# NightShade99/Self-Supervised-Vision

Measured on NVIDIA B200. Metric: ntxent_fwd_bwd_samples_per_s, higher is better.
Workload: dtype f16

## Files before the change

self-supervised-vision_b200/csrc/ntxent.cu:

```cuda
#include "sim_host.cuh"

using namespace ssvb;

namespace {

struct NtxPlan {
  int64_t n_glob, m, mpad, d, dpad;
  int mode;
  int normalize;
  float c, shift;
  float prescale;
  float wscale;
  float pos_c;
};

int make_plan(NtxPlan& pl, int64_t n_glob, int64_t d, int normalize, float temperature) {
  if (n_glob <= 0 || d <= 0 || !(temperature > 0.f)) return SSVB_ERR_INVALID;
  if (d % 4) return SSVB_ERR_ALIGNMENT;
  if (d > 256) return SSVB_ERR_UNSUPPORTED;
  if (2 * n_glob > (1 << 30)) return SSVB_ERR_UNSUPPORTED;
  pl.n_glob = n_glob;
  pl.m = 2 * n_glob;
  pl.mpad = sim_mpad(pl.m);
  pl.d = d;
  pl.dpad = sim_dpad(d);
  pl.normalize = normalize ? 1 : 0;
  const float c = SSVB_LOG2E / temperature;
  pl.mode = (normalize && 2.f * c <= 64.f) ? SIM_NTX_FIXED : SIM_NTX_ONLINE;
  if (pl.mode == SIM_NTX_FIXED) {
    pl.prescale = sqrtf(c);
    pl.c = 1.f;
    pl.shift = 0.f;
    pl.pos_c = 1.f;
    int k = 0;
    while ((int64_t{2} << k) <= pl.m) ++k;
    k -= 4;
    if (k < 0) k = 0;
    if (k > 14) k = 14;
    pl.wscale = static_cast<float>(1 << k);
  } else {
    pl.prescale = 1.f;
    pl.c = c;
    pl.shift = c;
    pl.pos_c = c;
    pl.wscale = 1.f;
  }
  return SSVB_OK;
}

struct SavedLayout {
  __nv_bfloat16* zhat;
  float* inv_norm;
  float* stat;
  size_t bytes;
};
SavedLayout saved_layout(void* base, int64_t mpad, int64_t dpad) {
  Carver c(base);
  SavedLayout s;
  s.zhat = c.take<__nv_bfloat16>(mpad * dpad);
  s.inv_norm = c.take<float>(mpad);
  s.stat = c.take<float>(mpad);
  s.bytes = c.used();
  return s;
}

struct WsLayout {
  float* pos;
  float* part_m;
  float* part_l;
  float* block_sums;
  unsigned int* counter;
  float* dacc;
  size_t bytes;
};
WsLayout ws_layout(void* base, int64_t local_rows, int64_t row_blocks, int64_t cols, int64_t dpad) {
  Carver c(base);
  WsLayout w;
  const int64_t lr = round_up(local_rows, 256);
  SimParams p{};
  p.row_blocks = static_cast<int>(row_blocks);
  p.cols = static_cast<int>(cols);
  plan_chunks(p, sim_fwd_bn(dpad), sim_fwd_min_tiles(dpad));
  size_t part_elems = static_cast<size_t>(4 * p.nchunks + 2) * lr;
  if (part_elems < static_cast<size_t>(sim_mpad(cols))) part_elems = sim_mpad(cols);
  w.pos = c.take<float>(lr);
  w.part_m = c.take<float>(part_elems);
  w.part_l = c.take<float>(part_elems);
  w.block_sums = c.take<float>(ceil_div(lr, 256) + 8);
  w.counter = c.take<unsigned int>(4);
  w.dacc = c.take<float>(lr * dpad);
  w.bytes = c.used();
  return w;
}

__global__ void ntx_grad_finish_kernel(const float* __restrict__ zi, const float* __restrict__ zj, int64_t ldi,
                                       int64_t ldj, int n_view, int d, int row0,
                                       const float* __restrict__ dacc, int ld_dacc,
                                       const __nv_bfloat16* __restrict__ zhat, int dpad,
                                       const float* __restrict__ inv_norm, int normalize, float inv_m_tau,
                                       const float* __restrict__ grad_out, float* __restrict__ dzi,
                                       float* __restrict__ dzj, int64_t ld_dzi, int64_t ld_dzj,
                                       float acc_scale, float zp_scale) {
  const int lrow = (blockIdx.x * blockDim.x + threadIdx.x) >> 5, lane = threadIdx.x & 31;
  if (lrow >= 2 * n_view) return;
  const int view = lrow >= n_view;
  const int r = lrow - view * n_view;
  const int a_glob = row0 + lrow;
  const int partner = view ? a_glob - n_view : a_glob + n_view;
  const float* z = view ? zj + static_cast<int64_t>(r) * ldj : zi + static_cast<int64_t>(r) * ldi;
  float* out = view ? dzj + static_cast<int64_t>(r) * ld_dzj : dzi + static_cast<int64_t>(r) * ld_dzi;
  const float scale = inv_m_tau * __ldg(grad_out);
  const float inv = normalize ? inv_norm[lrow] : 1.f;
  float g[2][4] = {{0.f, 0.f, 0.f, 0.f}, {0.f, 0.f, 0.f, 0.f}}, zh[2][4] = {{0.f, 0.f, 0.f, 0.f}, {0.f, 0.f, 0.f, 0.f}};
  float dot = 0.f;
#pragma unroll
  for (int it = 0; it < 2; ++it) {
    const int k = it * 128 + lane * 4;
    if (k < d) {
      const float4 acc = *reinterpret_cast<const float4*>(dacc + static_cast<int64_t>(lrow) * ld_dacc + k);
      const uint2 pz = *reinterpret_cast<const uint2*>(zhat + static_cast<int64_t>(partner) * dpad + k);
      const float2 p01 = unpack_h2(pz.x, normalize != 0), p23 = unpack_h2(pz.y, normalize != 0);
      const float4 zz = *reinterpret_cast<const float4*>(z + k);
      const float za = -2.f * zp_scale;
      g[it][0] = fmaf(acc.x, acc_scale, za * p01.x) * scale;
      g[it][1] = fmaf(acc.y, acc_scale, za * p01.y) * scale;
      g[it][2] = fmaf(acc.z, acc_scale, za * p23.x) * scale;
      g[it][3] = fmaf(acc.w, acc_scale, za * p23.y) * scale;
      zh[it][0] = zz.x * inv; zh[it][1] = zz.y * inv; zh[it][2] = zz.z * inv; zh[it][3] = zz.w * inv;
    }
    dot += g[it][0] * zh[it][0] + g[it][1] * zh[it][1] + g[it][2] * zh[it][2] + g[it][3] * zh[it][3];
  }
  if (normalize) {
    dot = warp_sum(dot);
#pragma unroll
    for (int it = 0; it < 2; ++it)
#pragma unroll
      for (int i = 0; i < 4; ++i) g[it][i] = (g[it][i] - dot * zh[it][i]) * inv;
  }
#pragma unroll
  for (int it = 0; it < 2; ++it) {
    const int k = it * 128 + lane * 4;
    if (k < d) *reinterpret_cast<float4*>(out + k) = make_float4(g[it][0], g[it][1], g[it][2], g[it][3]);
  }
}

int check_rows(const void* p, int64_t ld) {
  if (!p) return SSVB_ERR_INVALID;
  if ((reinterpret_cast<uintptr_t>(p) & 15) || (ld & 3)) return SSVB_ERR_ALIGNMENT;
  return SSVB_OK;
}

void fill_sim_params_rows(SimParams& p, const NtxPlan& pl, int nseg, int64_t seg_rows, int64_t s0, int64_t s1) {
  p = SimParams{};
  p.opf16 = pl.normalize ? 1 : 0;
  p.nseg = nseg;
  p.seg_rows = static_cast<int>(seg_rows);
  p.seg_start[0] = static_cast<int>(s0);
  p.seg_start[1] = static_cast<int>(s1);
  p.bps = static_cast<int>(ceil_div(seg_rows, 128));
  p.row_blocks = nseg * p.bps;
  p.cols = static_cast<int>(pl.m);
  p.c = pl.c;
  p.shift = pl.shift;
}

}

extern "C" {

int64_t ssvb_ntxent_dpad(int64_t d) { return sim_dpad(d); }
int64_t ssvb_ntxent_mpad(int64_t n_global) { return sim_mpad(2 * n_global); }

size_t ssvb_ntxent_saved_bytes(int64_t n, int64_t d) {
  if (n <= 0 || d <= 0) return 0;
  return saved_layout(nullptr, sim_mpad(2 * n), sim_dpad(d)).bytes;
}
size_t ssvb_ntxent_workspace_bytes(int64_t n, int64_t d) {
  if (n <= 0 || d <= 0) return 0;
  return ws_layout(nullptr, 2 * n, ceil_div(2 * n, 128), 2 * n, sim_dpad(d)).bytes;
}

int ssvb_ntxent_fwd(const float* zi, const float* zj, int64_t n, int64_t d, int64_t ld_zi, int64_t ld_zj,
                    int normalize, float temperature, float* loss, void* saved, void* workspace,
                    size_t workspace_bytes, void* stream) {
  SSVB_TRY(check_device_sm100());
  NtxPlan pl;
  SSVB_TRY(make_plan(pl, n, d, normalize, temperature));
  SSVB_TRY(check_rows(zi, ld_zi));
  SSVB_TRY(check_rows(zj, ld_zj));
  if (!loss || !saved || !workspace) return SSVB_ERR_INVALID;
  if (workspace_bytes < ssvb_ntxent_workspace_bytes(n, d)) return SSVB_ERR_WORKSPACE;
  cudaStream_t s = static_cast<cudaStream_t>(stream);
  SavedLayout sv = saved_layout(saved, pl.mpad, pl.dpad);
  WsLayout ws = ws_layout(workspace, pl.m, ceil_div(pl.m, 128), pl.m, pl.dpad);

  if (pl.mpad > pl.m)
    SSVB_CUDA(cudaMemsetAsync(sv.zhat + pl.m * pl.dpad, 0, (pl.mpad - pl.m) * pl.dpad * sizeof(__nv_bfloat16), s));
  {
    const int wpb = 8;
    pair_prep_kernel<<<static_cast<unsigned>(ceil_div(n, wpb)), wpb * 32, 0, s>>>(
        zi, zj, static_cast<int>(n), static_cast<int>(d), ld_zi, ld_zj, normalize, normalize ? 1 : 0, sv.zhat,
        sv.zhat + n * pl.dpad,
        static_cast<int>(pl.dpad), sv.inv_norm, sv.inv_norm + n, ws.pos, ws.pos + n, -1, pl.prescale, ws.counter);
    SSVB_LAUNCH_CHECK();
  }
  SimParams p;
  fill_sim_params_rows(p, pl, 1, pl.m, 0, 0);
  plan_chunks(p, sim_fwd_bn(pl.dpad), sim_fwd_min_tiles(pl.dpad));
  p.part_m = ws.part_m;
  p.part_l = ws.part_l;
  p.part_stride = static_cast<int>(round_up(pl.m, 256));
#ifdef SSVB_DBG_TIMING
  if (const char* e = getenv("SSVB_DBG_PTR")) p.dbg = reinterpret_cast<unsigned long long*>(strtoull(e, nullptr, 0));
#endif
  SSVB_TRY(launch_sim_fwd(pl.mode, sv.zhat, pl.mpad, sv.zhat, pl.mpad, pl.dpad, p, s));
  {
    const unsigned grid = static_cast<unsigned>(ceil_div(pl.m, 256));
    const float scale = 1.f / static_cast<float>(pl.m);
    if (pl.mode == SIM_NTX_FIXED)
      lse_finalize_kernel<SIM_NTX_FIXED><<<grid, 256, 0, s>>>(ws.part_m, ws.part_l, 4 * p.nchunks, p.part_stride,
                                                            static_cast<int>(pl.m), ws.pos, pl.c, pl.shift,
                                                            sv.stat, nullptr, ws.block_sums, ws.counter, scale, loss,
                                                            nullptr, nullptr, 0, 0, pl.wscale);
    else
      lse_finalize_kernel<SIM_NTX_ONLINE><<<grid, 256, 0, s>>>(ws.part_m, ws.part_l, 4 * p.nchunks, p.part_stride,
                                                             static_cast<int>(pl.m), ws.pos, pl.c, pl.shift,
                                                             sv.stat, nullptr, ws.block_sums, ws.counter, scale, loss);
    SSVB_LAUNCH_CHECK();
    if (pl.mpad > pl.m) {
      const float padv = pl.mode == SIM_NTX_FIXED ? 0.f : 1e30f;
      fill_kernel<<<static_cast<unsigned>(ceil_div(pl.mpad - pl.m, 256)), 256, 0, s>>>(sv.stat + pl.m,
                                                                                       pl.mpad - pl.m, padv);
      SSVB_LAUNCH_CHECK();
    }
  }
  return SSVB_OK;
}

int ssvb_ntxent_bwd(const float* zi, const float* zj, int64_t n, int64_t d, int64_t ld_zi, int64_t ld_zj,
                    int normalize, float temperature, const float* grad_out, const void* saved, float* dzi,
                    float* dzj, int64_t ld_dzi, int64_t ld_dzj, void* workspace, size_t workspace_bytes,
                    void* stream) {
  SSVB_TRY(check_device_sm100());
  NtxPlan pl;
  SSVB_TRY(make_plan(pl, n, d, normalize, temperature));
  SSVB_TRY(check_rows(zi, ld_zi));
  SSVB_TRY(check_rows(zj, ld_zj));
  SSVB_TRY(check_rows(dzi, ld_dzi));
  SSVB_TRY(check_rows(dzj, ld_dzj));
  if (!grad_out || !saved || !workspace) return SSVB_ERR_INVALID;
  if (workspace_bytes < ssvb_ntxent_workspace_bytes(n, d)) return SSVB_ERR_WORKSPACE;
  cudaStream_t s = static_cast<cudaStream_t>(stream);
  SavedLayout sv = saved_layout(const_cast<void*>(saved), pl.mpad, pl.dpad);
  WsLayout ws = ws_layout(workspace, pl.m, ceil_div(pl.m, 128), pl.m, pl.dpad);

  SimParams p;
  fill_sim_params_rows(p, pl, 1, pl.m, 0, 0);
  plan_chunks(p, 128, 8);
  p.rowstat = sv.stat;
  p.colstat = sv.stat;
  p.dacc = ws.dacc;
  p.ld_dacc = static_cast<int>(pl.dpad);
  p.use_atomic = p.nchunks > 1;
#ifdef SSVB_DBG_TIMING
  if (const char* e = getenv("SSVB_DBG_PTR")) p.dbg = reinterpret_cast<unsigned long long*>(strtoull(e, nullptr, 0));
#endif
  if (p.use_atomic) SSVB_CUDA(cudaMemsetAsync(ws.dacc, 0, pl.m * pl.dpad * sizeof(float), s));
  SSVB_TRY(launch_sim_bwd(pl.mode, sv.zhat, pl.mpad, sv.zhat, pl.mpad, pl.dpad, p, s));
  {
    const int wpb = 8;
    ntx_grad_finish_kernel<<<static_cast<unsigned>(ceil_div(pl.m, wpb)), wpb * 32, 0, s>>>(
        zi, zj, ld_zi, ld_zj, static_cast<int>(n), static_cast<int>(d), 0, ws.dacc,
        static_cast<int>(pl.dpad), sv.zhat, static_cast<int>(pl.dpad), sv.inv_norm, normalize,
        1.f / (static_cast<float>(pl.m) * temperature), grad_out, dzi, dzj, ld_dzi, ld_dzj,
        1.f / (pl.wscale * pl.prescale), 1.f / pl.prescale);
    SSVB_LAUNCH_CHECK();
  }
  return SSVB_OK;
}

size_t ssvb_ntxent_dist_workspace_bytes(int64_t world, int64_t n_local, int64_t d) {
  if (world <= 0 || n_local <= 0 || d <= 0) return 0;
  return ws_layout(nullptr, 2 * n_local, ceil_div(2 * n_local, 128), 2 * n_local * world, sim_dpad(d)).bytes;
}

namespace {
int dist_check(int64_t world, int64_t rank, int64_t n_local) {
  if (world <= 0 || rank < 0 || rank >= world || n_local <= 0) return SSVB_ERR_INVALID;
  return SSVB_OK;
}
}

int ssvb_ntxent_dist_prep(const float* zi, const float* zj, int64_t n_local, int64_t d, int64_t ld_zi,
                          int64_t ld_zj, int normalize, float temperature, int64_t world, int64_t rank,
                          void* zhat_all, float* inv_norm_local, float* pos_local, void* stream) {
  SSVB_TRY(check_device_sm100());
  SSVB_TRY(dist_check(world, rank, n_local));
  NtxPlan pl;
  SSVB_TRY(make_plan(pl, n_local * world, d, normalize, temperature));
  SSVB_TRY(check_rows(zi, ld_zi));
  SSVB_TRY(check_rows(zj, ld_zj));
  if (!zhat_all || !inv_norm_local || !pos_local) return SSVB_ERR_INVALID;
  cudaStream_t s = static_cast<cudaStream_t>(stream);
  __nv_bfloat16* zh = static_cast<__nv_bfloat16*>(zhat_all);
  if (pl.mpad > pl.m)
    SSVB_CUDA(cudaMemsetAsync(zh + pl.m * pl.dpad, 0, (pl.mpad - pl.m) * pl.dpad * sizeof(__nv_bfloat16), s));
  const int64_t row0 = rank * 2 * n_local;
  const int wpb = 8;
// ... 440 lines not shown
```

self-supervised-vision_b200/csrc/sim_host.cuh:

```cuda
#pragma once
#include "host_util.h"
#include "sim_kernels.cuh"

namespace ssvb {

inline int64_t sim_dpad(int64_t d) { return d <= 128 ? round_up(d, 64) : 256; }
inline int64_t sim_mpad(int64_t m) { return round_up(m, 256); }
inline int sim_fwd_bn(int64_t dpad) { return dpad > 128 ? 128 : kFwdBN; }
inline int sim_fwd_min_tiles(int64_t dpad) { return 1024 / sim_fwd_bn(dpad); }

inline void plan_chunks(SimParams& p, int BN, int min_tiles) {
  p.col_tiles = static_cast<int>(ceil_div(p.cols, BN));
  const int sms = num_sms();
  const int max_ch = p.col_tiles / min_tiles > 1 ? p.col_tiles / min_tiles : 1;
  int best = 1;
  double best_score = -1.0;
  for (int nch = 1; nch <= max_ch && nch <= 256; ++nch) {
    const int tpc = static_cast<int>(ceil_div(p.col_tiles, nch));
    const int real = static_cast<int>(ceil_div(p.col_tiles, tpc));
    if (real != nch) continue;
    const int64_t units = static_cast<int64_t>(p.row_blocks) * nch;
    const int64_t waves = ceil_div(units, sms);
    const double eff = static_cast<double>(p.row_blocks) * p.col_tiles / (static_cast<double>(waves) * sms * tpc);
    const double score = eff - 0.002 * nch;
    if (score > best_score) {
      best_score = score;
      best = nch;
    }
  }
  p.tiles_per_chunk = static_cast<int>(ceil_div(p.col_tiles, best));
  p.nchunks = static_cast<int>(ceil_div(p.col_tiles, p.tiles_per_chunk));
}

template <int KB, int MODE, bool OPF16 = false>
int launch_sim_fwd_t(const CUtensorMap& tmA, const CUtensorMap& tmB, const SimParams& p, cudaStream_t s) {
  auto kern = sim_fwd_kernel<KB, MODE, OPF16>;
  constexpr int smem = FwdCfg<KB>::SMEM;
  SSVB_TRY((set_smem_once<sim_fwd_kernel<KB, MODE, OPF16>>(smem)));
  const int nunits = p.row_blocks * p.nchunks;
  const int grid = nunits < num_sms() ? nunits : num_sms();
  const int slot = prof_begin(PROF_SIM_FWD, s);
  kern<<<grid, 640, smem, s>>>(tmA, tmB, p);
  prof_end(slot, s);
  SSVB_LAUNCH_CHECK();
  return SSVB_OK;
}
template <int KB, int MODE, bool OPF16 = false>
int launch_sim_bwd_t(const CUtensorMap& tmA, const CUtensorMap& tmB, const SimParams& p, cudaStream_t s) {
  auto kern = sim_bwd_kernel<KB, MODE, OPF16>;
  constexpr int smem = BwdCfg<KB>::SMEM;
  SSVB_TRY((set_smem_once<sim_bwd_kernel<KB, MODE, OPF16>>(smem)));
  const int nunits = p.row_blocks * p.nchunks;
  const int grid = nunits < num_sms() ? nunits : num_sms();
  const int slot = prof_begin(PROF_SIM_BWD, s);
  kern<<<grid, 640, smem, s>>>(tmA, tmB, p);
  prof_end(slot, s);
  SSVB_LAUNCH_CHECK();
  return SSVB_OK;
}

inline int launch_sim_fwd(int mode, const void* A, int64_t a_rows, const void* B, int64_t b_rows, int64_t dpad,
                          const SimParams& p, cudaStream_t s) {
  CUtensorMap tmA, tmB;
  SSVB_TRY(make_tmap_bf16(&tmA, A, a_rows, dpad, dpad, 128, p.opf16 != 0));
  SSVB_TRY(make_tmap_bf16(&tmB, B, b_rows, dpad, dpad, sim_fwd_bn(dpad), p.opf16 != 0));
  const int KB = static_cast<int>(dpad / 64);
#define SSVB_DISPATCH(KBV)                                                      \
  switch (mode) {                                                               \
    case SIM_NTX_FIXED:                                                         \
      if (p.opf16) return launch_sim_fwd_t<KBV, SIM_NTX_FIXED, true>(tmA, tmB, p, s);                   \
      return launch_sim_fwd_t<KBV, SIM_NTX_FIXED, false>(tmA, tmB, p, s);                               \
    case SIM_NTX_ONLINE:                                                        \
      if (p.opf16) return launch_sim_fwd_t<KBV, SIM_NTX_ONLINE, true>(tmA, tmB, p, s);                  \
      return launch_sim_fwd_t<KBV, SIM_NTX_ONLINE, false>(tmA, tmB, p, s);                              \
    case SIM_MOCO: return launch_sim_fwd_t<KBV, SIM_MOCO>(tmA, tmB, p, s);      \
    default: return SSVB_ERR_INVALID;                                           \
  }
  if (KB == 1) { SSVB_DISPATCH(1) }
  if (KB == 2) { SSVB_DISPATCH(2) }
  if (KB == 4) { SSVB_DISPATCH(4) }
#undef SSVB_DISPATCH
  return SSVB_ERR_UNSUPPORTED;
}
inline int launch_sim_bwd_half(int mode, const void* A, int64_t a_rows, const void* B, int64_t b_rows, int64_t dpad,
                               const SimParams& p, cudaStream_t s);
inline int launch_sim_bwd(int mode, const void* A, int64_t a_rows, const void* B, int64_t b_rows, int64_t dpad,
                          const SimParams& p, cudaStream_t s) {
  if (dpad <= 128) return launch_sim_bwd_half(mode, A, a_rows, B, b_rows, dpad, p, s);
  SimParams q = p;
  for (int h = 0; h < 2; ++h) {
    q.dhalf = h;
    SSVB_TRY(launch_sim_bwd_half(mode, A, a_rows, B, b_rows, dpad, q, s));
  }
  return SSVB_OK;
}
inline int launch_sim_bwd_half(int mode, const void* A, int64_t a_rows, const void* B, int64_t b_rows, int64_t dpad,
                          const SimParams& p, cudaStream_t s) {
  CUtensorMap tmA, tmB;
  SSVB_TRY(make_tmap_bf16(&tmA, A, a_rows, dpad, dpad, 128, p.opf16 != 0));
  SSVB_TRY(make_tmap_bf16(&tmB, B, b_rows, dpad, dpad, 128, p.opf16 != 0));
  const int KB = static_cast<int>(dpad / 64);
#define SSVB_DISPATCH(KBV)                                                      \
  switch (mode) {                                                               \
    case SIM_NTX_FIXED:                                                         \
      if (p.opf16) return launch_sim_bwd_t<KBV, SIM_NTX_FIXED, true>(tmA, tmB, p, s);  \
      return launch_sim_bwd_t<KBV, SIM_NTX_FIXED, false>(tmA, tmB, p, s);              \
    case SIM_NTX_ONLINE:                                                        \
      if (p.opf16) return launch_sim_bwd_t<KBV, SIM_NTX_ONLINE, true>(tmA, tmB, p, s); \
      return launch_sim_bwd_t<KBV, SIM_NTX_ONLINE, false>(tmA, tmB, p, s);             \
    case SIM_MOCO: return launch_sim_bwd_t<KBV, SIM_MOCO>(tmA, tmB, p, s);      \
    default: return SSVB_ERR_INVALID;                                           \
  }
  if (KB == 1) { SSVB_DISPATCH(1) }
  if (KB == 2) { SSVB_DISPATCH(2) }
// ... 244 lines not shown
```

self-supervised-vision_b200/csrc/sim_kernels.cuh:

```cuda
#pragma once
#include "common.cuh"

namespace ssvb {

enum SimMode { SIM_NTX_FIXED = 0, SIM_NTX_ONLINE = 1, SIM_MOCO = 2 };

struct SimParams {
  int nseg, seg_rows, seg_start[2];
  int bps;
  int row_blocks;
  int cols;
  int col_tiles;
  int nchunks, tiles_per_chunk;
  float c;
  float shift;
  float* part_m;
  float* part_l;
  int part_stride;
  const float* rowstat;
  const float* colstat;
  float* dacc;
  int ld_dacc;
  int use_atomic;
  unsigned long long* dbg;
  int opf16;
  int dhalf;
};

__device__ __forceinline__ uint8_t* align1024(uint8_t* p) {
  return reinterpret_cast<uint8_t*>((reinterpret_cast<uintptr_t>(p) + 1023) & ~static_cast<uintptr_t>(1023));
}

__device__ __forceinline__ void tmem_ld_wait_regs(uint32_t (&v)[32]) {
  asm volatile("tcgen05.wait::ld.sync.aligned;"
               : "+r"(v[0]), "+r"(v[1]), "+r"(v[2]), "+r"(v[3]), "+r"(v[4]), "+r"(v[5]), "+r"(v[6]), "+r"(v[7]),
                 "+r"(v[8]), "+r"(v[9]), "+r"(v[10]), "+r"(v[11]), "+r"(v[12]), "+r"(v[13]), "+r"(v[14]),
                 "+r"(v[15]), "+r"(v[16]), "+r"(v[17]), "+r"(v[18]), "+r"(v[19]), "+r"(v[20]), "+r"(v[21]),
                 "+r"(v[22]), "+r"(v[23]), "+r"(v[24]), "+r"(v[25]), "+r"(v[26]), "+r"(v[27]), "+r"(v[28]),
                 "+r"(v[29]), "+r"(v[30]), "+r"(v[31])::"memory");
}

struct UnitInfo {
  int g0;
  int lrow0;
  int nvalid;
  int t0, t1;
  int ch;
};
__device__ __forceinline__ UnitInfo decode_unit(const SimParams& p, int u) {
  UnitInfo ui;
  const int rb = u / p.nchunks;
  ui.ch = u - rb * p.nchunks;
  const int seg = rb / p.bps;
  const int rbi = rb - seg * p.bps;
  ui.g0 = p.seg_start[seg] + rbi * 128;
  ui.lrow0 = seg * p.seg_rows + rbi * 128;
  ui.nvalid = min(128, p.seg_rows - rbi * 128);
  ui.t0 = ui.ch * p.tiles_per_chunk;
  ui.t1 = min(p.col_tiles, ui.t0 + p.tiles_per_chunk);
  return ui;
}

#ifdef SSVB_DBG_TIMING
#define SSVB_T0() long long _t_prev = clock64()
#define SSVB_TP(slot) do { const long long _t_now = clock64(); _t_acc[slot] += _t_now - _t_prev; _t_prev = _t_now; } while (0)
#else
#define SSVB_T0() do {} while (0)
#define SSVB_TP(slot) do {} while (0)
#endif

__device__ __forceinline__ float ex2_poly3(float x);
#ifdef SSVB_DBG_NOEXP
#define SSVB_EX2(x) (x)
#else
#define SSVB_EX2(x) ex2f(x)
#endif
#ifndef SSVB_POLY_MOD_FWD
#define SSVB_POLY_MOD_FWD 3
#endif
#ifndef SSVB_POLY_FWD_MOD
#define SSVB_POLY_FWD_MOD 2
#endif
#ifndef SSVB_POLY_FWD_CNT
#define SSVB_POLY_FWD_CNT 1
#endif
#ifndef SSVB_POLY_BWD_MOD
#define SSVB_POLY_BWD_MOD 3
#endif
#ifndef SSVB_POLY_BWD_CNT
#define SSVB_POLY_BWD_CNT 1
#endif

__device__ __forceinline__ unsigned long long ex2_poly3_x2(unsigned long long x2) {
  const unsigned long long magic2 = pack_f32x2(12582912.f, 12582912.f);
  const unsigned long long nmagic2 = pack_f32x2(-12582912.f, -12582912.f);
  const unsigned long long r2 = add_f32x2(x2, magic2);
  const unsigned long long t2 = add_f32x2(r2, nmagic2);
  const unsigned long long f2 = fma_f32x2(t2, pack_f32x2(-1.f, -1.f), x2);
  unsigned long long q2 = fma_f32x2(f2, pack_f32x2(5.517166745e-2f, 5.517166745e-2f),
                                    pack_f32x2(2.426111221e-1f, 2.426111221e-1f));
  q2 = fma_f32x2(q2, f2, pack_f32x2(6.932609858e-1f, 6.932609858e-1f));
// ... 189 lines not shown
      const UnitInfo ui = decode_unit(p, u);
      mbar_wait(&a_full[0], ucount & 1);
      for (int t = ui.t0; t < ui.t1; ++t, ++gt) {
        const int st = gt % NSTAGE, buf = gt % NBUF;
        mbar_wait(&b_full[st], (gt / NSTAGE) & 1);
        mbar_wait(&s_empty[buf], ((gt / NBUF) & 1) ^ 1);
        tc_fence_after();
        if (elect_one()) {
          const uint32_t bbase = smem_u32(sB + st * C::B_BYTES);
#ifndef SSVB_DBG_FWD_NOS
#pragma unroll
          for (int kb = 0; kb < KB; ++kb)
#pragma unroll
            for (int k4 = 0; k4 < 4; ++k4)
              umma_ss(tmem + buf * BN, desc_kmajor(abase + kb * (128 * 128) + k4 * 32),
                      desc_kmajor(bbase + kb * (BN * 128) + k4 * 32), IDESC, (kb | k4) != 0);
#endif
          umma_commit(&b_empty[st]);
          umma_commit(&s_full[buf]);
          if (t == ui.t1 - 1) umma_commit(&a_empty[0]);
        }
        __syncwarp();
      }
    }
  }
  } else {
    asm volatile("setmaxnreg.inc.sync.aligned.u32 104;");
    const int wgi = (warp - 4) >> 2;
    const int pair = wgi >> 1, half = wgi & 1;
    const int q = warp & 3;
    const int row_l = q * 32 + lane;
    const uint32_t tlane = static_cast<uint32_t>(q * 32) << 16;
    int gt = 0;
    const int my_buf = NBUF == 2 ? pair : wgi;
    const uint32_t a_s_full = smem_u32(&s_full[my_buf]), a_s_empty = smem_u32(&s_empty[my_buf]);
#ifdef SSVB_DBG_TIMING
    long long _t_acc[8] = {0, 0, 0, 0, 0, 0, 0, 0};
#endif
    SSVB_T0();
    for (int u = blockIdx.x; u < nunits; u += gridDim.x) {
      const UnitInfo ui = decode_unit(p, u);
      const int a_glob = ui.g0 + row_l;
      float m = -1e30f;
      float l[4] = {0.f, 0.f, 0.f, 0.f};
      for (int t = ui.t0; t < ui.t1; ++t, ++gt) {
        if (NBUF == 2 ? ((gt & 1) != pair) : ((gt & 3) != wgi)) continue;
        const int buf = NBUF == 2 ? pair : wgi;
        SSVB_TP(0);
        mbar_wait_a(a_s_full, (gt / NBUF) & 1);
        tc_fence_after();
        SSVB_TP(1);
        const int j0 = t * BN + (NBUF == 2 ? half * 128 : 0);
        const bool special = (MODE != SIM_MOCO && j0 < ui.g0 + 128 && j0 + 128 > ui.g0) || (j0 + 128 > p.cols);
        const uint32_t taddr = tmem + tlane + buf * BN + (NBUF == 2 ? half * 128 : 0);
#ifdef SSVB_DBG_TIMING
        if (special)
          fwd_tile<MODE, true>(taddr, p, a_glob, j0, m, l, a_s_empty, lane, _t_acc, _t_prev);
        else
          fwd_tile<MODE, false>(taddr, p, a_glob, j0, m, l, a_s_empty, lane, _t_acc, _t_prev);
#else
        if (special)
          fwd_tile<MODE, true>(taddr, p, a_glob, j0, m, l, a_s_empty, lane);
        else
          fwd_tile<MODE, false>(taddr, p, a_glob, j0, m, l, a_s_empty, lane);
#endif
      }
      if (row_l < ui.nvalid) {
        const size_t o = static_cast<size_t>(ui.ch * 4 + wgi) * p.part_stride + ui.lrow0 + row_l;
        p.part_l[o] = (l[0] + l[1]) + (l[2] + l[3]);
        if (MODE != SIM_NTX_FIXED) p.part_m[o] = m;
      }
    }
#ifdef SSVB_DBG_TIMING
    if (p.dbg && blockIdx.x == 0 && warp == 4 && lane == 0)
      for (int i = 0; i < 8; ++i) p.dbg[16 + i] = static_cast<unsigned long long>(_t_acc[i]);
#endif
  }
  tc_fence_before();
  __syncthreads();
  if (warp == 2) tmem_dealloc<512>(tmem);
}

template <int KB>
struct BwdCfg {
  static constexpr int BN = 128;
  static constexpr int DP = (KB >= 2) ? 128 : 64;
  static constexpr int A_BYTES = 128 * 128 * KB;
  static constexpr int B_BYTES = BN * 128 * KB;
  static constexpr int CS_BYTES = BN * 4;
  static constexpr int NSTAGE = (KB == 1) ? 8 : (KB == 2 ? 5 : 2);
  static constexpr int NBARS = 2 + 2 * NSTAGE + 8 + 2;
  static constexpr int SMEM = 1024 + A_BYTES + NSTAGE * (B_BYTES + CS_BYTES) + NBARS * 8 + 16;
  static constexpr int T_S = 0;
  static constexpr int T_DZ = 256;
  static constexpr int T_W = 384;
};

__device__ __forceinline__ float ex2_poly3(float x) {
  const float magic = 12582912.f;
  const float r = x + magic;
  const float f = x - (r - magic);
  float p = fmaf(f, 5.517166745e-2f, 2.426111221e-1f);
  p = fmaf(p, f, 6.932609858e-1f);
  p = fmaf(p, f, 9.999280736e-1f);
  return __int_as_float(__float_as_int(p) + (__float_as_int(r) << 23));
}
#ifndef SSVB_POLY_MOD_BWD
#define SSVB_POLY_MOD_BWD 0
#endif

template <int MODE, bool MASKED, bool OPF16>
__device__ __forceinline__ void bwd_weights32(const uint32_t (&sv)[32], uint32_t (&pk)[16], const SimParams& p,
                                              int a_glob, int colbase, float rs, uint32_t cs32, float& wsum) {
#ifndef SSVB_BWD_SCALAR_MATH
  if (MODE == SIM_NTX_FIXED && !MASKED) {
    const unsigned long long rs2 = pack_f32x2(rs, rs);
#pragma unroll
    for (int i2 = 0; i2 < 8; ++i2) {
      unsigned long long cu[2];
      lds_v4(cs32 + i2 * 16, cu[0], cu[1]);
#pragma unroll
      for (int e = 0; e < 2; ++e) {
        const int i = i2 * 2 + e;
        const bool poly = (i % SSVB_POLY_BWD_MOD) < SSVB_POLY_BWD_CNT;
        unsigned long long e2;
        if (poly) {
          e2 = ex2_poly3_x2(pack_f32x2(__uint_as_float(sv[2 * i]), __uint_as_float(sv[2 * i + 1])));
        } else {
          e2 = pack_f32x2(SSVB_EX2(__uint_as_float(sv[2 * i])), SSVB_EX2(__uint_as_float(sv[2 * i + 1])));
        }
        const unsigned long long w2 = mul_f32x2(e2, add_f32x2(rs2, cu[e]));
        float w0, w1;
        unpack_f32x2(w2, w0, w1);
        pk[i] = pack_h2<OPF16>(w0, w1);
      }
    }
    return;
  }
#endif
#pragma unroll
  for (int i4 = 0; i4 < 8; ++i4) {
    float csv[4] = {0.f, 0.f, 0.f, 0.f};
    if (MODE != SIM_MOCO) {
      unsigned long long c01, c23;
      lds_v4(cs32 + i4 * 16, c01, c23);
      unpack_f32x2(c01, csv[0], csv[1]);
      unpack_f32x2(c23, csv[2], csv[3]);
    }
    float w[4];
#pragma unroll
    for (int e = 0; e < 4; ++e) {
      const int i = i4 * 4 + e;
      const float s = __uint_as_float(sv[i]);
      float wv;
      if (MODE == SIM_NTX_FIXED) {
        const float x = fmaf(s, p.c, -p.shift);
        const bool poly = !MASKED && SSVB_POLY_MOD_BWD > 0 && (i % (SSVB_POLY_MOD_BWD > 0 ? SSVB_POLY_MOD_BWD : 1)) == 1;
        wv = (poly ? ex2_poly3(x) : SSVB_EX2(x)) * (rs + csv[e]);
      } else if (MODE == SIM_NTX_ONLINE) {
        const float t = s * p.c;
        wv = ex2f(t - rs) + ex2f(t - csv[e]);
      } else {
        wv = ex2f(fmaf(s, p.c, -rs));
      }
      if (MASKED && MODE != SIM_MOCO && (colbase + i == a_glob)) wv = 0.f;
      if (MASKED && MODE == SIM_MOCO && (colbase + i >= p.cols)) wv = 0.f;
// ... 256 lines not shown
```

Measured before the change: 11.80 million.

## Exploit similarity-matrix symmetry in NT-Xent forward with banded tile kernel

Adds a symmetric forward kernel that computes only a band of roughly half the block tiles of the Z·Zᵀ similarity matrix. Each off-diagonal tile contributes row sums directly and column sums through a shared-memory reduction written to extra partial buffers, which the LSE finalize step then merges. The aim is to cut tensor-core and exp work nearly in half for the fixed-shift mode with dpad up to 128. The cost is more workspace, extra column-reduction traffic and barriers, and more complex masking logic.

```diff
diff --git a/self-supervised-vision_b200/csrc/ntxent.cu b/self-supervised-vision_b200/csrc/ntxent.cu
--- a/self-supervised-vision_b200/csrc/ntxent.cu
+++ b/self-supervised-vision_b200/csrc/ntxent.cu
@@ -82,6 +82,13 @@
   p.cols = static_cast<int>(cols);
   plan_chunks(p, sim_fwd_bn(dpad), sim_fwd_min_tiles(dpad));
   size_t part_elems = static_cast<size_t>(4 * p.nchunks + 2) * lr;
+  if (local_rows == cols && dpad <= 128) {
+    SimParams q{};
+    q.row_blocks = static_cast<int>(row_blocks);
+    const int ncol = plan_sym(q);
+    const size_t sym_elems = static_cast<size_t>(4 * q.nchunks + ncol) * lr;
+    if (part_elems < sym_elems) part_elems = sym_elems;
+  }
   if (part_elems < static_cast<size_t>(sim_mpad(cols))) part_elems = sim_mpad(cols);
   w.pos = c.take<float>(lr);
   w.part_m = c.take<float>(part_elems);
@@ -206,24 +213,33 @@
   }
   SimParams p;
   fill_sim_params_rows(p, pl, 1, pl.m, 0, 0);
-  plan_chunks(p, sim_fwd_bn(pl.dpad), sim_fwd_min_tiles(pl.dpad));
   p.part_m = ws.part_m;
   p.part_l = ws.part_l;
   p.part_stride = static_cast<int>(round_up(pl.m, 256));
 #ifdef SSVB_DBG_TIMING
   if (const char* e = getenv("SSVB_DBG_PTR")) p.dbg = reinterpret_cast<unsigned long long*>(strtoull(e, nullptr, 0));
 #endif
-  SSVB_TRY(launch_sim_fwd(pl.mode, sv.zhat, pl.mpad, sv.zhat, pl.mpad, pl.dpad, p, s));
+  int nparts;
+  if (pl.mode == SIM_NTX_FIXED && pl.dpad <= 128) {
+    const int ncol = plan_sym(p);
+    p.colpart = ws.part_l + static_cast<size_t>(4 * p.nchunks) * p.part_stride;
+    nparts = 4 * p.nchunks + ncol;
+    SSVB_TRY(launch_sim_fwd_sym(sv.zhat, pl.mpad, pl.dpad, p, s));
+  } else {
+    plan_chunks(p, sim_fwd_bn(pl.dpad), sim_fwd_min_tiles(pl.dpad));
+    nparts = 4 * p.nchunks;
+    SSVB_TRY(launch_sim_fwd(pl.mode, sv.zhat, pl.mpad, sv.zhat, pl.mpad, pl.dpad, p, s));
+  }
   {
     const unsigned grid = static_cast<unsigned>(ceil_div(pl.m, 256));
     const float scale = 1.f / static_cast<float>(pl.m);
     if (pl.mode == SIM_NTX_FIXED)
-      lse_finalize_kernel<SIM_NTX_FIXED><<<grid, 256, 0, s>>>(ws.part_m, ws.part_l, 4 * p.nchunks, p.part_stride,
+      lse_finalize_kernel<SIM_NTX_FIXED><<<grid, 256, 0, s>>>(ws.part_m, ws.part_l, nparts, p.part_stride,
                                                             static_cast<int>(pl.m), ws.pos, pl.c, pl.shift,
                                                             sv.stat, nullptr, ws.block_sums, ws.counter, scale, loss,
                                                             nullptr, nullptr, 0, 0, pl.wscale);
     else
-      lse_finalize_kernel<SIM_NTX_ONLINE><<<grid, 256, 0, s>>>(ws.part_m, ws.part_l, 4 * p.nchunks, p.part_stride,
+      lse_finalize_kernel<SIM_NTX_ONLINE><<<grid, 256, 0, s>>>(ws.part_m, ws.part_l, nparts, p.part_stride,
                                                              static_cast<int>(pl.m), ws.pos, pl.c, pl.shift,
                                                              sv.stat, nullptr, ws.block_sums, ws.counter, scale, loss);
     SSVB_LAUNCH_CHECK();
diff --git a/self-supervised-vision_b200/csrc/sim_host.cuh b/self-supervised-vision_b200/csrc/sim_host.cuh
--- a/self-supervised-vision_b200/csrc/sim_host.cuh
+++ b/self-supervised-vision_b200/csrc/sim_host.cuh
@@ -9,8 +9,8 @@
 inline int sim_fwd_bn(int64_t dpad) { return dpad > 128 ? 128 : kFwdBN; }
 inline int sim_fwd_min_tiles(int64_t dpad) { return 1024 / sim_fwd_bn(dpad); }
 
-inline void plan_chunks(SimParams& p, int BN, int min_tiles) {
-  p.col_tiles = static_cast<int>(ceil_div(p.cols, BN));
+inline void plan_chunks_tiles(SimParams& p, int col_tiles, int min_tiles) {
+  p.col_tiles = col_tiles;
   const int sms = num_sms();
   const int max_ch = p.col_tiles / min_tiles > 1 ? p.col_tiles / min_tiles : 1;
   int best = 1;
@@ -30,6 +30,34 @@
   }
   p.tiles_per_chunk = static_cast<int>(ceil_div(p.col_tiles, best));
   p.nchunks = static_cast<int>(ceil_div(p.col_tiles, p.tiles_per_chunk));
+}
+inline void plan_chunks(SimParams& p, int BN, int min_tiles) {
+  plan_chunks_tiles(p, static_cast<int>(ceil_div(p.cols, BN)), min_tiles);
+}
+inline int plan_sym(SimParams& p) {
+  p.band = p.row_blocks / 2 + 1;
+  plan_chunks_tiles(p, (p.band + 1) / 2, sim_fwd_min_tiles(128));
+  return (p.row_blocks - 1) / 2;
+}
+
+template <int KB>
+int launch_sim_fwd_sym_t(const CUtensorMap& tmA, const CUtensorMap& tmB, const SimParams& p, cudaStream_t s) {
+  auto kern = sim_fwd_sym_kernel<KB, true>;
+  constexpr int smem = SymCfg<KB>::SMEM;
+  SSVB_TRY((set_smem_once<sim_fwd_sym_kernel<KB, true>>(smem)));
+  const int nunits = p.row_blocks * p.nchunks;
+  const int grid = nunits < num_sms() ? nunits : num_sms();
+  const int slot = prof_begin(PROF_SIM_FWD, s);
+  kern<<<grid, 640, smem, s>>>(tmA, tmB, p);
+  prof_end(slot, s);
+  SSVB_LAUNCH_CHECK();
+  return SSVB_OK;
+}
+inline int launch_sim_fwd_sym(const void* Z, int64_t z_rows, int64_t dpad, const SimParams& p, cudaStream_t s) {
+  if (!p.opf16 || dpad > 128) return SSVB_ERR_UNSUPPORTED;
+  CUtensorMap tm;
+  SSVB_TRY(make_tmap_bf16(&tm, Z, z_rows, dpad, dpad, 128, true));
+  return dpad == 64 ? launch_sim_fwd_sym_t<1>(tm, tm, p, s) : launch_sim_fwd_sym_t<2>(tm, tm, p, s);
 }
 
 template <int KB, int MODE, bool OPF16 = false>
diff --git a/self-supervised-vision_b200/csrc/sim_kernels.cuh b/self-supervised-vision_b200/csrc/sim_kernels.cuh
--- a/self-supervised-vision_b200/csrc/sim_kernels.cuh
+++ b/self-supervised-vision_b200/csrc/sim_kernels.cuh
@@ -17,6 +17,8 @@
   float* part_m;
   float* part_l;
   int part_stride;
+  int band;
+  float* colpart;
   const float* rowstat;
   const float* colstat;
   float* dacc;
@@ -372,6 +374,276 @@
 }
 
 template <int KB>
+struct SymCfg {
+  static constexpr int BN = 256;
+  static constexpr int A_BYTES = 128 * 128 * KB;
+  static constexpr int B_BYTES = BN * 128 * KB;
+  static constexpr int NSTAGE = (KB == 1) ? 4 : 2;
+  static constexpr int CP_BYTES = 4 * 16384;
+  static constexpr int NBARS = 4 + 2 * NSTAGE + 4;
+  static constexpr int SMEM = 1024 + A_BYTES + NSTAGE * B_BYTES + CP_BYTES + NBARS * 8 + 16;
+};
+
+__device__ __forceinline__ void tmem_ld_16x256b_x4(uint32_t taddr, uint32_t* v) {
+  asm volatile(
+      "tcgen05.ld.sync.aligned.16x256b.x4.b32 "
+      "{%0, %1, %2, %3, %4, %5, %6, %7, %8, %9, %10, %11, %12, %13, %14, %15}, [%16];"
+      : "=r"(v[0]), "=r"(v[1]), "=r"(v[2]), "=r"(v[3]), "=r"(v[4]), "=r"(v[5]), "=r"(v[6]), "=r"(v[7]),
+        "=r"(v[8]), "=r"(v[9]), "=r"(v[10]), "=r"(v[11]), "=r"(v[12]), "=r"(v[13]), "=r"(v[14]), "=r"(v[15])
+      : "r"(taddr)
+      : "memory");
+}
+__device__ __forceinline__ void named_bar_sync(int id, int nthreads) {
+  asm volatile("bar.sync %0, %1;" ::"r"(id), "r"(nthreads) : "memory");
+}
+
+template <bool MASKED, bool COLS>
+__device__ __forceinline__ void sym_tile(uint32_t taddr, const SimParams& p, unsigned long long (&racc)[4],
+                                         uint32_t a_s_empty, int lane, uint32_t cp_st0, uint32_t cp_st1, int barid,
+                                         int row_w, int col_t, bool diag) {
+  uint32_t v[2][32];
+  tmem_ld_16x256b_x4(taddr, v[0]);
+  tmem_ld_16x256b_x4(taddr + (16u << 16), v[0] + 16);
+  const int g = lane >> 2, c4 = lane & 3;
+#pragma unroll
+  for (int cc = 0; cc < 4; ++cc) {
+    uint32_t(&cur)[32] = v[cc & 1];
+    tmem_ld_wait_regs(cur);
+    if (cc < 3) {
+      tmem_ld_16x256b_x4(taddr + (cc + 1) * 32, v[(cc + 1) & 1]);
+      tmem_ld_16x256b_x4(taddr + (16u << 16) + (cc + 1) * 32, v[(cc + 1) & 1] + 16);
+    } else {
+      tc_fence_before();
+      __syncwarp();
+      if (lane == 0) mbar_arrive_a(a_s_empty);
+    }
+    unsigned long long cacc[4];
+#pragma unroll
+    for (int k = 0; k < 4; ++k) {
+#pragma unroll
+      for (int r = 0; r < 4; ++r) {
+        const int idx = 16 * (r >> 1) + 4 * k + 2 * (r & 1);
+        unsigned long long e2;
+        if (MASKED) {
+          const int row = row_w + g + 8 * r, col = col_t + cc * 32 + 8 * k + 2 * c4;
+          float e[2];
+#pragma unroll
+          for (int j = 0; j < 2; ++j) {
+            const bool off = (diag && row == col + j) || row >= p.cols || col + j >= p.cols;
+            e[j] = ex2f(off ? -INFINITY : __uint_as_float(cur[idx + j]));
+          }
+          e2 = pack_f32x2(e[0], e[1]);
+        } else if (((4 * k + r) % SSVB_POLY_FWD_MOD) < SSVB_POLY_FWD_CNT) {
+          e2 = ex2_poly3_x2(pack_f32x2(__uint_as_float(cur[idx]), __uint_as_float(cur[idx + 1])));
+        } else {
+          e2 = pack_f32x2(SSVB_EX2(__uint_as_float(cur[idx])), SSVB_EX2(__uint_as_float(cur[idx + 1])));
+        }
+        racc[r] = add_f32x2(racc[r], e2);
+        if (COLS) cacc[k] = r == 0 ? e2 : add_f32x2(cacc[k], e2);
+      }
+    }
+    if (COLS) {
+      if (cc == 0) named_bar_sync(barid, 128);
+      const uint32_t o = cc * 4096;
+      asm volatile("st.shared.v2.b64 [%0], {%1, %2};" ::"r"(cp_st0 + o), "l"(cacc[0]), "l"(cacc[1]) : "memory");
+      asm volatile("st.shared.v2.b64 [%0], {%1, %2};" ::"r"(cp_st1 + o), "l"(cacc[2]), "l"(cacc[3]) : "memory");
+    }
+  }
+}
+
+template <int KB, bool OPF16>
+__global__ void __launch_bounds__(640, 1)
+sim_fwd_sym_kernel(const __grid_constant__ CUtensorMap tmA, const __grid_constant__ CUtensorMap tmB, const SimParams p) {
+  using C = SymCfg<KB>;
+  constexpr int BN = C::BN, NSTAGE = C::NSTAGE, NBUF = 2;
+  extern __shared__ uint8_t smem_raw[];
+  uint8_t* smem = align1024(smem_raw);
+  uint8_t* sA = smem;
+  uint8_t* sB = smem + C::A_BYTES;
+  uint8_t* sCP = sB + NSTAGE * C::B_BYTES;
+  uint64_t* bars = reinterpret_cast<uint64_t*>(sCP + C::CP_BYTES);
+  uint64_t* a_full = bars;
+  uint64_t* a_empty = bars + 2;
+  uint64_t* b_full = bars + 4;
+  uint64_t* b_empty = b_full + NSTAGE;
+  uint64_t* s_full = b_empty + NSTAGE;
+  uint64_t* s_empty = s_full + NBUF;
+  uint32_t* tmem_slot = reinterpret_cast<uint32_t*>(s_empty + NBUF);
+
+  const int warp = threadIdx.x >> 5, lane = threadIdx.x & 31;
+  const int R = p.row_blocks;
+  if (warp == 0 && lane == 0) {
+    tma_prefetch_desc(&tmA);
+    tma_prefetch_desc(&tmB);
+  }
+  if (warp == 1 && lane == 0) {
+    mbar_init(&a_full[0], 1);
+    mbar_init(&a_empty[0], 1);
+    for (int i = 0; i < NBUF; ++i) {
+      mbar_init(&s_full[i], 1);
+      mbar_init(&s_empty[i], 8);
+    }
+    for (int i = 0; i < NSTAGE; ++i) {
+      mbar_init(&b_full[i], 1);
+      mbar_init(&b_empty[i], 1);
+    }
+    fence_barrier_init();
+  }
+  if (warp == 2) tmem_alloc<512>(tmem_slot);
+  tc_fence_before();
+  __syncthreads();
+  tc_fence_after();
+  const uint32_t tmem = *tmem_slot;
+  const int nunits = p.row_blocks * p.nchunks;
+
+  if (warp < 4) {
+    asm volatile("setmaxnreg.dec.sync.aligned.u32 40;");
+    if (warp == 0) {
+      int ucount = 0, gt = 0;
+      for (int u = blockIdx.x; u < nunits; u += gridDim.x, ++ucount) {
+        const UnitInfo ui = decode_unit(p, u);
+        const int rb = ui.g0 >> 7;
+        mbar_wait(&a_empty[0], (ucount & 1) ^ 1);
+        if (elect_one()) {
+          mbar_expect_tx(&a_full[0], C::A_BYTES);
+#pragma unroll
+          for (int kb = 0; kb < KB; ++kb) tma_load_2d(sA + kb * (128 * 128), &tmA, &a_full[0], kb * 64, ui.g0);
+        }
+        __syncwarp();
+        for (int t = ui.t0; t < ui.t1; ++t, ++gt) {
+          const int st = gt % NSTAGE;
+          mbar_wait(&b_empty[st], ((gt / NSTAGE) & 1) ^ 1);
+          if (elect_one()) {
+            mbar_expect_tx(&b_full[st], C::B_BYTES);
+#pragma unroll
+            for (int h = 0; h < 2; ++h) {
+              const int b = (rb + 2 * t + h) % R;
+#pragma unroll
+              for (int kb = 0; kb < KB; ++kb)
+                tma_load_2d(sB + st * C::B_BYTES + kb * (BN * 128) + h * (128 * 128), &tmB, &b_full[st], kb * 64,
+                            b * 128);
+            }
+          }
+          __syncwarp();
+        }
+      }
+    } else if (warp == 1) {
+      constexpr uint32_t IDESC = make_idesc(128, BN, 0, 0, OPF16 ? 0 : 1);
+      const uint32_t abase = smem_u32(sA);
+      int ucount = 0, gt = 0;
+      for (int u = blockIdx.x; u < nunits; u += gridDim.x, ++ucount) {
+        const UnitInfo ui = decode_unit(p, u);
+        mbar_wait(&a_full[0], ucount & 1);
+        for (int t = ui.t0; t < ui.t1; ++t, ++gt) {
+          const int st = gt % NSTAGE, buf = gt % NBUF;
+          mbar_wait(&b_full[st], (gt / NSTAGE) & 1);
+          mbar_wait(&s_empty[buf], ((gt / NBUF) & 1) ^ 1);
+          tc_fence_after();
+          if (elect_one()) {
+            const uint32_t bbase = smem_u32(sB + st * C::B_BYTES);
+#pragma unroll
+            for (int kb = 0; kb < KB; ++kb)
+#pragma unroll
+              for (int k4 = 0; k4 < 4; ++k4)
+                umma_ss(tmem + buf * BN, desc_kmajor(abase + kb * (128 * 128) + k4 * 32),
+                        desc_kmajor(bbase + kb * (BN * 128) + k4 * 32), IDESC, (kb | k4) != 0);
+            umma_commit(&b_empty[st]);
+            umma_commit(&s_full[buf]);
+            if (t == ui.t1 - 1) umma_commit(&a_empty[0]);
+          }
+          __syncwarp();
+        }
+      }
+    }
+  } else {
+    asm volatile("setmaxnreg.inc.sync.aligned.u32 104;");
+    const int wgi = (warp - 4) >> 2;
+    const int pair = wgi >> 1, half = wgi & 1;
+    const int q = warp & 3;
+    const int g = lane >> 2, c4 = lane & 3;
+    const uint32_t tlane = static_cast<uint32_t>(q * 32) << 16;
+    const uint32_t a_s_full = smem_u32(&s_full[pair]), a_s_empty = smem_u32(&s_empty[pair]);
+    const int barid = 1 + wgi;
+    const uint32_t cp_wg = smem_u32(sCP) + wgi * 16384;
+    const uint32_t cp_st = cp_wg + (q * 8 + g) * 128 + c4 * 32;
+    const uint32_t cp_st0 = cp_st + ((g & 1) << 4), cp_st1 = cp_st + (((g & 1) ^ 1) << 4);
+    const int H = (R - 1) >> 1;
+    const bool ragged = (p.cols & 127) != 0;
+    int gt = 0;
+    for (int u = blockIdx.x; u < nunits; u += gridDim.x) {
+      const UnitInfo ui = decode_unit(p, u);
+      const int rb = ui.g0 >> 7;
+      unsigned long long racc[4] = {0ull, 0ull, 0ull, 0ull};
+      for (int t = ui.t0; t < ui.t1; ++t, ++gt) {
+        if ((gt & 1) != pair) continue;
+        mbar_wait_a(a_s_full, (gt >> 1) & 1);
+        tc_fence_after();
+        const int o = 2 * t + half;
+        const uint32_t taddr = tmem + tlane + pair * BN + half * 128;
+        if (o >= p.band) {
+          tc_fence_before();
+          __syncwarp();
+          if (lane == 0) mbar_arrive_a(a_s_empty);
+          continue;
+        }
+        const int b = (rb + o) % R;
+        const bool cols = o >= 1 && o <= H;
+        const bool masked = o == 0 || (ragged && (rb == R - 1 || b == R - 1));
+        const int row_w = ui.g0 + q * 32;
+        if (!cols) {
+          sym_tile<true, false>(taddr, p, racc, a_s_empty, lane, 0, 0, barid, row_w, b * 128, o == 0);
+          continue;
+        }
+        if (masked)
+          sym_tile<true, true>(taddr, p, racc, a_s_empty, lane, cp_st0, cp_st1, barid, row_w, b * 128, false);
+        else
+          sym_tile<false, true>(taddr, p, racc, a_s_empty, lane, cp_st0, cp_st1, barid, row_w, b * 128, false);
+        named_bar_sync(barid, 128);
+        if (q < 2) {
+          const int rd = q * 32 + lane;
+          const int rd_k = (rd >> 2) & 3;
+          const uint32_t cp_rd = cp_wg + (rd >> 4) * 4096 + (rd & 3) * 32;
+          const int rd_col = (rd >> 4) * 32 + 8 * rd_k + 2 * (rd & 3);
+          unsigned long long s2 = pack_f32x2(0.f, 0.f);
+#pragma unroll
+          for (int w = 0; w < 4; ++w)
+#pragma unroll
+            for (int gg = 0; gg < 8; ++gg) {
+              unsigned long long x;
+              asm volatile("ld.shared.b64 %0, [%1];"
+                           : "=l"(x)
+                           : "r"(cp_rd + (w * 8 + gg) * 128 + ((rd_k * 8) ^ ((gg & 1) << 4))));
+              s2 = add_f32x2(s2, x);
+            }
+          float c0, c1;
+          unpack_f32x2(s2, c0, c1);
+          *reinterpret_cast<float2*>(p.colpart + static_cast<size_t>(o - 1) * p.part_stride + b * 128 + rd_col) =
+              make_float2(c0, c1);
+        }
+      }
+      float rs[4];
+#pragma unroll
+      for (int r = 0; r < 4; ++r) {
+        float x0, x1;
+        unpack_f32x2(racc[r], x0, x1);
+        rs[r] = x0 + x1;
+        rs[r] += __shfl_xor_sync(0xffffffffu, rs[r], 1);
+        rs[r] += __shfl_xor_sync(0xffffffffu, rs[r], 2);
+      }
+#pragma unroll
+      for (int r = 0; r < 4; ++r) {
+        const int row_l = q * 32 + g + 8 * r;
+        if (c4 == r && row_l < ui.nvalid)
+          p.part_l[static_cast<size_t>(ui.ch * 4 + wgi) * p.part_stride + ui.lrow0 + row_l] = rs[r];
+      }
+    }
+  }
+  tc_fence_before();
+  __syncthreads();
+  if (warp == 2) tmem_dealloc<512>(tmem);
+}
+
+template <int KB>
 struct BwdCfg {
   static constexpr int BN = 128;
   static constexpr int DP = (KB >= 2) ? 128 : 64;
```

Measured after the change: 13.77 million (median of 6 runs). +16.8%, better.
